# yanzq95/DHD

Hardware: AMD Instinct MI355X
Metric: samples/sec (6-cam fwd+bwd) DHD-S view-transform hot path (higher is better)
Workload: dtype f32

## Files before the change

dhd_amd/csrc/sfa_stage.hip:

```cpp
#include <stdlib.h>

#include <type_traits>

#include "sfa_gemm_cu.h"
#include "sfa_half.h"
#include "sfa_mfma.h"

using namespace dhd_sfa;

namespace {

constexpr int kEwBlock = 256;
constexpr int kPlaneChunks = 4;
constexpr int kPwBlock = 256;
constexpr int kPwStep = 16;
constexpr int kWgBlock = 512;
constexpr int kWgStride = 33;
constexpr int kWgWorkers = 256;
__host__ __device__ inline long long wg_first_step(long long n, long long w, long long W) { return n * w / W; }
__host__ __device__ inline int wg_owner(long long n, long long s, long long W) { return (int)(((s + 1) * W + n - 1) / n) - 1; }
inline int wgrad_blocks(int c) { const int ot = c == 128 ? 128 : 256; return (c / ot) * (c / ot); }
inline int wgrad_workers(int c) { const int nob = wgrad_blocks(c); return kWgWorkers / nob > 0 ? kWgWorkers / nob : 1; }
constexpr int kBwdFoldDefault = 3;

__device__ __forceinline__ float block_sum(float v, float* sm) {
  v = group_sum(v, DHD_WAVE);
  const int lane = threadIdx.x & 63, wv = threadIdx.x >> 6;
  __syncthreads();
  if (lane == 0) sm[wv] = v;
  __syncthreads();
  float t = 0.f;
  for (int k = 0; k < (int)(blockDim.x / DHD_WAVE); ++k) t += sm[k];
  return t;
}

template <class TS> constexpr bool kHalfStorage = !std::is_same_v<TS, float>;
template <class TS> constexpr bool kStreamAll = kHalfStorage<TS>;
template <class TS> constexpr int kWideInFlight = kHalfStorage<TS> ? 2 : 1;
template <class TS> constexpr bool kFoldPairwise = !kHalfStorage<TS>;

template <int N> __device__ __forceinline__ void chunk_range(int hw, int* lo, int* hi) {
  static_assert(N == 4 || N == 8, "16 bytes of float32 or of a half type");
  const int n = hw >> (N == 8 ? 3 : 2), per = (n + kPlaneChunks - 1) / kPlaneChunks;
  *lo = blockIdx.x * per;
  *hi = min(n, *lo + per);
}

template <class TO, int N> struct IoVec {
  static constexpr bool k16 = N == kVec16<TO>;
  static_assert(k16 || (N == 4 && sizeof(TO) == 2), "16 bytes, or four elements of a half type");
  using raw = std::conditional_t<k16, raw16<TO>, u32x2>;
  static __device__ __forceinline__ raw ld(const TO* base, size_t i) { return __builtin_nontemporal_load(reinterpret_cast<const raw*>(base) + i); }
  static __device__ __forceinline__ void widen(raw w, float* v) {
    if constexpr (k16) {
      widen16<TO>(w, v);
    } else {
      const f32x2 a = Pair<TO>::widen(w.x), b = Pair<TO>::widen(w.y);
      v[0] = a.x; v[1] = a.y; v[2] = b.x; v[3] = b.y;
    }
  }
  static __device__ __forceinline__ void store(TO* base, size_t i, const float* v) {
    if constexpr (k16) {
      Vec16<TO, true>::store(base, i, v);
    } else {
      typedef TO t4 __attribute__((ext_vector_type(4)));
      const t4 h = {(TO)v[0], (TO)v[1], (TO)v[2], (TO)v[3]};
      __builtin_nontemporal_store(h, reinterpret_cast<t4*>(base) + i);
    }
  }
};

template <int N> __device__ __forceinline__ float tree_sum(const float* v) {
  if constexpr (N == 4) return (v[0] + v[1]) + (v[2] + v[3]);
  else return tree_sum<N / 2>(v) + tree_sum<N / 2>(v + N / 2);
}

template <class TS> __device__ __forceinline__ float fold_sum(float acc, const float* a) {
  if constexpr (kFoldPairwise<TS>) return acc + tree_sum<kVec16<TS>>(a);
#pragma unroll
  for (int j = 0; j < kVec16<TS>; ++j) acc += a[j];
  return acc;
}
template <class TS, class D> __device__ __forceinline__ float fold_dot(float acc, const float* a, D d) {
  if constexpr (kFoldPairwise<TS>) {
    static_assert(kVec16<TS> == 4, "the pairwise fold is written for four elements");
    return acc + ((a[0] * d(0) + a[1] * d(1)) + (a[2] * d(2) + a[3] * d(3)));
  }
#pragma unroll
  for (int j = 0; j < kVec16<TS>; ++j) acc = fmaf(a[j], d(j), acc);
  return acc;
}

template <int K, class Load, class Body> __device__ __forceinline__ void for_each_vector(int lo, int hi, Load load, Body body) {
  int i = lo + threadIdx.x;
  if constexpr (K == 2) {
    for (; i + kEwBlock < hi; i += 2 * kEwBlock) {
      const auto u = load(i), w = load(i + kEwBlock);
      body(u, i);
      body(w, i + kEwBlock);
    }
    if (i < hi) body(load(i), i);
  } else {
    for (; i < hi; i += kEwBlock) body(load(i), i);
  }
}


template <class TS>
__device__ __forceinline__ void plane_mean_block(const TS* __restrict__ x, float* __restrict__ part, int hw, float* sm) {
  constexpr int N = kVec16<TS>;
  using X = Vec16<TS, true>;
  const size_t plane = blockIdx.y;
  const TS* p = x + plane * hw;
  int lo, hi;
  chunk_range<N>(hw, &lo, &hi);
  float a0 = 0.f, a1 = 0.f;
  int i = lo + threadIdx.x;
  for (; i + kEwBlock < hi; i += 2 * kEwBlock) {
    float v[N], w[N];
    X::load(p, i, v);
    X::load(p, (size_t)i + kEwBlock, w);
    a0 += tree_sum<N>(v);
    a1 += tree_sum<N>(w);
  }
  if (i < hi) {
    float v[N];
    X::load(p, i, v);
    a0 += tree_sum<N>(v);
  }
  const float tot = block_sum(a0 + a1, sm);
  if (threadIdx.x == 0) part[plane * kPlaneChunks + blockIdx.x] = tot;
}

__global__ __launch_bounds__(kEwBlock) void plane_mean_kernel(const float* __restrict__ x, float* __restrict__ part, int hw) {
  __shared__ float sm[kEwBlock / DHD_WAVE];
  plane_mean_block(x, part, hw, sm);
}

constexpr int kFcBlock = 1024;
__global__ __launch_bounds__(kFcBlock) void fc_forward_kernel(const float* __restrict__ part, const float* __restrict__ w1,
                                                              const float* __restrict__ b1, const float* __restrict__ w2,
                                                              const float* __restrict__ b2, float* __restrict__ s,
                                                              float* __restrict__ hbuf, float* __restrict__ a,
                                                              float* __restrict__ tab, int c, int r, int hw,
                                                              int* __restrict__ ticks, int n_ticks) {
  extern __shared__ float sh[];
  if (blockIdx.x == 0)
    for (int i = threadIdx.x; i < n_ticks; i += kFcBlock) ticks[i] = 0;
  float* ss = sh;
  float* hh = sh + 2 * c;
  const int b = blockIdx.x, c2 = 2 * c;
  for (int i = threadIdx.x; i < c2; i += kFcBlock) {
    const float* q = part + ((size_t)b * c2 + i) * kPlaneChunks;
    float v = ((q[0] + q[1]) + (q[2] + q[3])) / (float)hw;
    ss[i] = v;
    s[(size_t)b * c2 + i] = v;
  }
  __syncthreads();
  const int lane = threadIdx.x & 63, wv = threadIdx.x >> 6;
  for (int j0 = wv * 4; j0 < r; j0 += 4 * (kFcBlock / DHD_WAVE)) {
    float acc[4] = {0.f, 0.f, 0.f, 0.f};
    for (int i = lane; i < c2; i += DHD_WAVE) {
      const float sv = ss[i];
#pragma unroll
      for (int q = 0; q < 4; ++q)
        if (j0 + q < r) acc[q] = fmaf(w1[(size_t)(j0 + q) * c2 + i], sv, acc[q]);
    }
#pragma unroll
    for (int q = 0; q < 4; ++q) {
      const float t = group_sum(acc[q], DHD_WAVE);
      if (lane == 0 && j0 + q < r) {
        const float v = fmaxf(t + b1[j0 + q], 0.f);
        hh[j0 + q] = v;
        hbuf[(size_t)b * r + j0 + q] = v;
      }
    }
// ... 1337 lines not shown
      constexpr int OT = decltype(ot_c)::value;
      if constexpr (!std::is_same<TS, float>::value) {
        const size_t shmem = (size_t)2 * 4 * 2 * (OT / 32) * 64 * 16;
        return launch_lds<pw_wgrad_h_kernel<TS, OT, V::two, V::relu>>(grid, block, shmem, shmem, st, a0, a1, acoef, a_bs, b0, b1, bcoef,
                                                                     b_bs, partial, c, hw, b, workers);
      } else if (p.wgrad == Wgrad::w3) {
        const size_t shmem = (size_t)2 * 2 * 2 * (OT / 32) * 2 * 64 * 16;
        if (fold.mode != 0) {
          if (nob != 1 || fold.mode != (V::two ? 2 : 1)) return (int)DHD_EUNSUPPORTED;
          return launch_lds<pw_wgrad3_kernel<OT, false, V::two, V::relu, V::two ? 2 : 1>>(grid, block, shmem, shmem, st, a0, a1, acoef, a_bs, b0, b1,
                                                                                         bcoef, b_bs, partial, c, hw, b, workers, fold.aux,
                                                                                         fold.mean, fold.rows);
        }
        return launch_lds<pw_wgrad3_kernel<OT, true, V::two, V::relu>>(grid, block, shmem, shmem, st, a0, a1, acoef, a_bs, b0, b1, bcoef,
                                                                      b_bs, partial, c, hw, b, workers, static_cast<const float*>(nullptr),
                                                                      static_cast<const float*>(nullptr), static_cast<float*>(nullptr));
      } else if (p.wgrad == Wgrad::w6) {
        const size_t shmem = (size_t)2 * 2 * (OT / 32) * 3 * 64 * 16;
        return launch_lds<pw_wgrad6_kernel<OT, true, V::two, V::relu>>(grid, block, shmem, shmem, st, a0, a1, acoef, a_bs, b0, b1, bcoef,
                                                                      b_bs, partial, c, hw, b, workers);
      } else {
        const size_t shmem = (size_t)4 * OT * kWgStride * sizeof(float);
        return launch_lds<pw_wgrad_kernel<OT, true, V::two, V::relu>>(grid, block, shmem, shmem, st, a0, a1, acoef, a_bs, b0, b1, bcoef,
                                                                     b_bs, partial, c, hw, b, workers);
      }
    };
    return ot == 128 ? run(IntC<128>{}) : run(IntC<256>{});
  });
  if (rc != DHD_OK) return rc;
  const int n = c * c;
  hipLaunchKernelGGL(wgrad_reduce_kernel, dim3(dhd_cdiv(n, DHD_WAVE)), dim3(kEwBlock), 0, st, partial, gw, n, workers);
  DHD_LAUNCH_CHECK();
  return DHD_OK;
}

template <class TS>
int launch_mean_pack(const Plan& p, const TS* x, const float* w1, const float* w2, void* const dst[4], float* mean_part, int b,
                     int c, int hw, hipStream_t st) {
  const int blocks_each = dhd_cdiv((c / 32) * (c / 16) * 64, kEwBlock);
  if (p.pack == Pack::cu || p.pack == Pack::res || p.pack == Pack::cuh) {
    PackJob job;
    job.w[0] = w1; job.w[1] = w2;
    for (int i = 0; i < 4; ++i) job.dst[i] = static_cast<u32x4*>(dst[i]);
    job.c = c; job.nt = p.nt; job.cob = p.cob; job.cu = p.pack == Pack::cu ? 1 : 0;
    job.blocks_each = blocks_each;
    const dim3 grid(kPlaneChunks, b * 2 * c + dhd_cdiv(4 * blocks_each, kPlaneChunks));
    hipLaunchKernelGGL(plane_mean_pack_kernel<TS>, grid, dim3(kEwBlock), 0, st, x, mean_part, hw, b * 2 * c, job);
    DHD_LAUNCH_CHECK();
    return DHD_OK;
  }
  if constexpr (std::is_same_v<TS, float>) {
    hipLaunchKernelGGL(plane_mean_kernel, dim3(kPlaneChunks, b * 2 * c), dim3(kEwBlock), 0, st, x, mean_part, hw);
    DHD_LAUNCH_CHECK();
    for (int i = 0; i < 4; ++i) {
      const float* wi = i & 1 ? w2 : w1;
      if (p.pack == Pack::six)
        hipLaunchKernelGGL(pack_weight6_kernel, dim3(blocks_each), dim3(kEwBlock), 0, st, wi, i >> 1, static_cast<u32x4*>(dst[i]), c, p.cot);
      else
        hipLaunchKernelGGL(pack_weight_kernel, dim3(dhd_cdiv(c * c, kEwBlock)), dim3(kEwBlock), 0, st, wi, i >> 1, static_cast<float*>(dst[i]),
                           c, p.cot);
      DHD_LAUNCH_CHECK();
    }
    return DHD_OK;
  }
  return DHD_EINVAL;
}

template <class TS, class TO>
int stage_forward(const Plan& p, const TS* x, const dhd_sfa_weights* w, TO* out, void* saved, void* scratch, int b, int c, int hw,
                  int lo, int hi, double* sync, hipStream_t st) {
  const int r = w->hidden;
  const SavedLayout S = saved_layout(b, c, hw, r, p.storage);
  const ScratchLayout T = scratch_layout(b, c, hw, r, p.storage);
  char* sv = static_cast<char*>(saved);
  char* sc = static_cast<char*>(scratch);
  auto SF = [&](size_t off) { return reinterpret_cast<float*>(sv + off); };
  auto TF = [&](size_t off) { return reinterpret_cast<float*>(sc + off); };
  TS* y1 = reinterpret_cast<TS*>(sv + S.y1);
  TS* y2 = reinterpret_cast<TS*>(sv + S.y2);
  float* stat_part = p.fused_stats ? TF(T.stat_part) : nullptr;
  const dim3 planes(kPlaneChunks, b * c), per_ch(dhd_cdiv(c, kEwBlock));
  const size_t cs = (size_t)c * hw;
  int stat_rows = 0, rc;
  struct Bn {
    const float *shift, *gamma, *beta;
    float *run_mean, *run_var;
    float momentum, eps;
    long long* batches;
    float *mean, *rstd, *scsh;
    double* loc;
  };
  const Bn bn1 = {w->conv1_b, w->bn1_w, w->bn1_b, w->bn1_mean, w->bn1_var, w->momentum1, w->eps1,
                  reinterpret_cast<long long*>(w->bn1_batches), SF(S.mean1), SF(S.rstd1), SF(S.scsh1), reinterpret_cast<double*>(sv + S.loc1)};
  const Bn bn2 = {w->conv2_b, w->bn2_w, w->bn2_b, w->bn2_mean, w->bn2_var, w->momentum2, w->eps2,
                  reinterpret_cast<long long*>(w->bn2_batches), SF(S.mean2), SF(S.rstd2), SF(S.scsh2), reinterpret_cast<double*>(sv + S.loc2)};
  auto publish = [&](const Bn& n, float* tab) {
    hipLaunchKernelGGL(bn_stats_finalize_kernel, dim3(c / 4), dim3(kEwBlock), 0, st, TF(T.stat_part), stat_rows, n.shift, n.gamma, n.beta,
                       n.run_mean, n.run_var, n.momentum, n.eps, n.mean, n.rstd, n.scsh, tab, b, c, hw, sync, n.loc, nullptr, nullptr);
  };
  auto coef = [&](const Bn& n, const TS* y, float* tab) {
    if (!w->training) {
      hipLaunchKernelGGL(bn_eval_coef_kernel, per_ch, dim3(kEwBlock), 0, st, n.gamma, n.beta, n.run_mean, n.run_var, n.eps, n.mean, n.rstd,
                         n.scsh, tab, b, c);
    } else if (p.fused_stats) {
      hipLaunchKernelGGL(bn_stats_finalize_kernel, dim3(c / 4), dim3(kEwBlock), 0, st, TF(T.stat_part), stat_rows, n.shift, n.gamma, n.beta,
                         n.run_mean, n.run_var, n.momentum, n.eps, n.mean, n.rstd, n.scsh, tab, b, c, hw, nullptr, nullptr, sync, n.batches);
    } else if constexpr (std::is_same<TS, float>::value) {
      hipLaunchKernelGGL(moments_kernel, planes, dim3(kEwBlock), 0, st, y, TF(T.part), c, hw);
      hipLaunchKernelGGL(bn_train_finalize_kernel, per_ch, dim3(kEwBlock), 0, st, TF(T.part), b * kPlaneChunks, y, hw, n.gamma, n.beta,
                         n.run_mean, n.run_var, n.momentum, n.eps, n.mean, n.rstd, n.scsh, tab, b, c, hw, n.batches);
    }
  };
  if (sync && !p.fused_stats) return DHD_EUNSUPPORTED;

  if (lo <= 0) {
    void* const dst[4] = {sc + T.wp1, sc + T.wp2, sv + S.wp1t, sv + S.wp2t};
    rc = launch_mean_pack(p, x, w->conv1_w, w->conv2_w, dst, TF(T.mean_part), b, c, hw, st);
    if (rc != DHD_OK) return rc;
    hipLaunchKernelGGL(fc_forward_kernel, dim3(b), dim3(kFcBlock), (size_t)(2 * c + r) * sizeof(float), st, TF(T.mean_part), w->fc1_w,
                       w->fc1_b, w->fc2_w, w->fc2_b, SF(S.s), SF(S.h), SF(S.a1), SF(S.tab_a), c, r, hw, reinterpret_cast<int*>(sv + S.tick),
                       2 * c + kTickWords);
    DHD_LAUNCH_CHECK();
    rc = launch_gemm(p, GemmCall<TS>{kConv1, x, x + cs, 2 * cs, c, SF(S.tab_a), sc + T.wp1, w->conv1_b, nullptr, stat_part, y1},
                     b, c, hw, st, &stat_rows);
    if (rc != DHD_OK) return rc;
    if (sync) {
      publish(bn1, SF(S.tab1));
      DHD_LAUNCH_CHECK();
    }
  }
  if (hi <= 0) return DHD_OK;
  if (lo <= 1) {
    coef(bn1, y1, SF(S.tab1));
    DHD_LAUNCH_CHECK();
    rc = launch_gemm(p, GemmCall<TS>{kConv2, y1, nullptr, cs, c, SF(S.tab1), sc + T.wp2, w->conv2_b,
                                     reinterpret_cast<unsigned*>(sv + S.mask), stat_part, y2},
                     b, c, hw, st, &stat_rows);
    if (rc != DHD_OK) return rc;
    if (sync) {
      publish(bn2, TF(T.tab_g2));
      DHD_LAUNCH_CHECK();
    }
  }
  if (hi <= 1) return DHD_OK;
  coef(bn2, y2, TF(T.tab_g2));
  hipLaunchKernelGGL((blend2_bn_kernel<TS, TO>), planes, dim3(kEwBlock), 0, st, x, SF(S.a1), y2, SF(S.scsh2), out, c, hw);
  DHD_LAUNCH_CHECK();
  return DHD_OK;
}

int bwd_fold_mode() {
  static const int mode = [] {
    const char* e = getenv("DHD_SFA_BWD_FOLD");
    return e != nullptr && e[0] >= '0' && e[0] <= '3' && e[1] == 0 ? e[0] - '0' : kBwdFoldDefault;
  }();
  return mode;
}

template <class TS, class TO>
int stage_backward(const Plan& p, const TS* x, const dhd_sfa_weights* w, const void* saved, const TO* gout, TO* gx,
                   const dhd_sfa_grads* grads, void* scratch, int b, int c, int hw, int lo, int hi, double* sync, hipStream_t st) {
  const int r = w->hidden;
  const SavedLayout S = saved_layout(b, c, hw, r, p.storage);
  const ScratchLayout T = scratch_layout(b, c, hw, r, p.storage);
  char* sv = const_cast<char*>(static_cast<const char*>(saved));
  char* sc = static_cast<char*>(scratch);
  auto SF = [&](size_t off) { return reinterpret_cast<float*>(sv + off); };
  auto TF = [&](size_t off) { return reinterpret_cast<float*>(sc + off); };
  const TS* y1 = reinterpret_cast<const TS*>(sv + S.y1);
  const TS* y2 = reinterpret_cast<const TS*>(sv + S.y2);
  TS* g2 = reinterpret_cast<TS*>(sc + T.g2);
  TS* g1 = reinterpret_cast<TS*>(sc + T.g1);
  TS* du = reinterpret_cast<TS*>(sc + T.du);
  unsigned* mask = reinterpret_cast<unsigned*>(sv + S.mask);
  int* tick = reinterpret_cast<int*>(sv + S.tick);
  const dim3 planes(kPlaneChunks, b * c), per_ch(dhd_cdiv(c, kEwBlock));
  const size_t cs = (size_t)c * hw;
  int rc;
  const BnTail tail2 = {sync ? nullptr : tick, w->bn2_w, SF(S.mean2), SF(S.rstd2), TF(T.tab_g2), grads->bn2_w, grads->bn2_b,
                        grads->conv2_b, w->training, b, hw};
  const BnTail tail1 = {sync ? nullptr : tick + c, w->bn1_w, SF(S.mean1), SF(S.rstd1), TF(T.tab_g1), grads->bn1_w, grads->bn1_b,
                        grads->conv1_b, w->training, b, hw};
  auto coef_out = [&](const BnTail& t) {
    hipLaunchKernelGGL(bn_backward_coef_kernel, per_ch, dim3(kEwBlock), 0, st, TF(T.part), t.gamma, t.mean, t.rstd, w->training, t.tab,
                       t.dgamma, t.dbeta, t.dbias, b, c, hw, sync, nullptr, nullptr, nullptr);
  };
  auto coef_in = [&](const BnTail& t, size_t loc, const float* bias) {
    hipLaunchKernelGGL(bn_backward_coef_kernel, per_ch, dim3(kEwBlock), 0, st, TF(T.part), t.gamma, t.mean, t.rstd, w->training, t.tab,
                       t.dgamma, t.dbeta, t.dbias, b, c, hw, nullptr, sync, reinterpret_cast<const double*>(sv + loc), bias);
  };
  if (sync && !p.fused_stats) return DHD_EUNSUPPORTED;
  int fold = 0;
  const int fold_workers = wgrad_workers(c);
  if constexpr (std::is_same_v<TS, float>) {
    const size_t plane = (size_t)b * cs * sizeof(float);
    if (p.gemm == Gemm::cu && p.wgrad == Wgrad::w3 && sync == nullptr && wgrad_blocks(c) == 1 && (size_t)fold_workers * 2 * c * sizeof(float) <= plane &&
        (size_t)(fold_workers + b) * c * sizeof(float) <= plane)
      fold = bwd_fold_mode();
  }
  float* rows1 = reinterpret_cast<float*>(du);
  float* rows2 = reinterpret_cast<float*>(g2);

  if (lo <= 0) {
    hipLaunchKernelGGL((blend2_bn_bwd_kernel<TS, TO>), planes, dim3(kEwBlock), 0, st, x, SF(S.a1), y2, SF(S.scsh2), SF(S.mean2), gout, g2, TF(T.part),
                       TF(T.da1), c, hw, tail2);
    if (sync) coef_out(tail2);
    DHD_LAUNCH_CHECK();
  }
  if (hi <= 0) return DHD_OK;
  if (lo <= 1) {
    if (sync) coef_in(tail2, S.loc2, w->conv2_b);
    DHD_LAUNCH_CHECK();
  }
  if (lo <= 1 && (fold & 1)) {
    if constexpr (std::is_same_v<TS, float>) {
      rc = launch_gemm(p, GemmCall<TS>{kDgrad2, g2, y2, cs, c, TF(T.tab_g2), sv + S.wp2t, nullptr, mask, nullptr, g1, y1, SF(S.scsh1), CuBlend{}, 0, g2},
                       b, c, hw, st);
      if (rc != DHD_OK) return rc;
      rc = launch_wgrad<TS>(p, kConv2, g2, nullptr, nullptr, cs, y1, nullptr, SF(S.tab1), cs, TF(T.wpart), grads->conv2_w, b, c, hw, st,
                            WgradFold{1, g1, SF(S.mean1), rows1});
      if (rc != DHD_OK) return rc;
      const BnRowsJob j1 = {tail1.gamma, tail1.mean, tail1.rstd, tail1.tab, tail1.dgamma, tail1.dbeta, tail1.dbias, w->training, b, hw};
      hipLaunchKernelGGL(bn_backward_rows_kernel, dim3(c / 4), dim3(kEwBlock), 0, st, rows1, fold_workers, j1, c);
      DHD_LAUNCH_CHECK();
    }
  } else if (lo <= 1) {
    rc = launch_wgrad<TS>(p, kConv2, g2, y2, TF(T.tab_g2), cs, y1, nullptr, SF(S.tab1), cs, TF(T.wpart), grads->conv2_w, b, c, hw, st);
    if (rc != DHD_OK) return rc;
    rc = launch_gemm(p, GemmCall<TS>{kDgrad2, g2, y2, cs, c, TF(T.tab_g2), sv + S.wp2t, nullptr, mask, nullptr, g1, y1, SF(S.scsh1)},
                     b, c, hw, st);
    if (rc != DHD_OK) return rc;
    hipLaunchKernelGGL(pair_sums_kernel<TS>, planes, dim3(kEwBlock), 0, st, g1, y1, SF(S.mean1), TF(T.part), c, hw, tail1);
    if (sync) coef_out(tail1);
    DHD_LAUNCH_CHECK();
  }
  if (hi <= 1) return DHD_OK;
  if (sync) coef_in(tail1, S.loc1, w->conv1_b);
  DHD_LAUNCH_CHECK();
  if (fold & 2) {
    if constexpr (std::is_same_v<TS, float>) {
      rc = launch_gemm(p, GemmCall<TS>{kDgrad1, g1, y1, cs, c, TF(T.tab_g1), sv + S.wp1t, nullptr, nullptr, nullptr, du, nullptr, nullptr, CuBlend{}, 0, g1},
                       b, c, hw, st);
      if (rc != DHD_OK) return rc;
      rc = launch_wgrad<TS>(p, kConv1, g1, nullptr, nullptr, cs, x, x + cs, SF(S.tab_a), 2 * cs, TF(T.wpart), grads->conv1_w, b, c, hw, st,
                            WgradFold{2, du, nullptr, rows2});
      if (rc != DHD_OK) return rc;
      hipLaunchKernelGGL(fc_backward_kernel, dim3(b), dim3(kEwBlock), (size_t)(c + r + kEwBlock) * sizeof(float), st, TF(T.da1), rows2,
                         SF(S.a1), SF(S.h), w->fc1_w, w->fc2_w, TF(T.dpre2), TF(T.dh), TF(T.ds), c, r, fold_workers, (hw + 31) / 32);
    }
  } else {
    rc = launch_wgrad<TS>(p, kConv1, g1, y1, TF(T.tab_g1), cs, x, x + cs, SF(S.tab_a), 2 * cs, TF(T.wpart), grads->conv1_w, b, c, hw, st);
    if (rc != DHD_OK) return rc;
    rc = launch_gemm(p, GemmCall<TS>{kDgrad1, g1, y1, cs, c, TF(T.tab_g1), sv + S.wp1t, nullptr, nullptr, nullptr, du}, b, c, hw, st);
    if (rc != DHD_OK) return rc;
    hipLaunchKernelGGL(blend1_da_kernel<TS>, planes, dim3(kEwBlock), 0, st, x, du, TF(T.da2), c, hw);
    hipLaunchKernelGGL(fc_backward_kernel, dim3(b), dim3(kEwBlock), (size_t)(c + r + kEwBlock) * sizeof(float), st, TF(T.da1), TF(T.da2),
                       SF(S.a1), SF(S.h), w->fc1_w, w->fc2_w, TF(T.dpre2), TF(T.dh), TF(T.ds), c, r, 0, 0);
  }
  const int n_fc = r * 2 * c + c * r + r + c;
  const FcGradJob fcj = {TF(T.dpre2), TF(T.dh), SF(S.h), SF(S.s), grads->fc1_w, grads->fc1_b, grads->fc2_w, grads->fc2_b, b, r};
  const int fc_rows = dhd_cdiv(dhd_cdiv(n_fc, kEwBlock), kPlaneChunks);
  const dim3 planes_fc(kPlaneChunks, b * c + fc_rows);
  hipLaunchKernelGGL((stage_gx_kernel<TS, TO>), planes_fc, dim3(kEwBlock), 0, st, SF(S.a1), y2, SF(S.scsh2), gout, du, TF(T.ds), gx, c, hw, fc_rows, fcj);
  DHD_LAUNCH_CHECK();
  return DHD_OK;
}

inline bool infer_form_exists(const Plan& p, int form) {
  switch (form) {
    case DHD_SFA_INFER_AUTO: case DHD_SFA_INFER_UNFUSED: return true;
    case DHD_SFA_INFER_TWO_PASS: return p.gemm == Gemm::cu || p.gemm == Gemm::cuh;
    case DHD_SFA_INFER_ONE_PASS: return p.gemm == Gemm::cuh;
    default: return false;
  }
}
inline int infer_resolve(const Plan& p, int form) {
  if (form != DHD_SFA_INFER_AUTO) return form;
  if (infer_form_exists(p, DHD_SFA_INFER_ONE_PASS)) return DHD_SFA_INFER_ONE_PASS;
  return infer_form_exists(p, DHD_SFA_INFER_TWO_PASS) ? DHD_SFA_INFER_TWO_PASS : DHD_SFA_INFER_UNFUSED;
}

struct InferLayout {
  size_t wp1, wp2, mean_part, s, h, a1, tab_a, mean1, rstd1, scsh1, tab1, mean2, rstd2, scsh2, tab2, y1, total;
};
inline InferLayout infer_layout(int b, int c, int hw, int r, int storage, bool with_y1) {
  const bool half = storage != DHD_F32;
  const size_t cc = (size_t)c * c;
  InferLayout L;
  size_t o = 0;
  auto take = [&](size_t bytes) { size_t at = o; o += (bytes + 255) & ~(size_t)255; return at; };
  auto f = [&](size_t n) { return take(n * sizeof(float)); };
  L.wp1 = take(half ? 2 * cc : 8 * cc); L.wp2 = take(half ? 2 * cc : 8 * cc);
  L.mean_part = f((size_t)b * 2 * c * kPlaneChunks);
  L.s = f((size_t)b * 2 * c); L.h = f((size_t)b * r); L.a1 = f((size_t)b * c); L.tab_a = f((size_t)b * 3 * c);
  L.mean1 = f(c); L.rstd1 = f(c); L.scsh1 = f(2 * c); L.tab1 = f((size_t)b * 3 * c);
  L.mean2 = f(c); L.rstd2 = f(c); L.scsh2 = f(2 * c); L.tab2 = f((size_t)b * 3 * c);
  L.y1 = take(with_y1 ? (size_t)b * c * hw * (half ? 2 : 4) : 0);
  L.total = o;
  return L;
}

inline size_t infer_scratch_total(const Plan& p, int form, int b, int c, int hw, int r) {
  const int f = infer_resolve(p, form);
  if (f != DHD_SFA_INFER_UNFUSED) return infer_layout(b, c, hw, r, p.storage, f == DHD_SFA_INFER_TWO_PASS).total;
  return saved_layout(b, c, hw, r, p.storage).total + scratch_layout(b, c, hw, r, p.storage).total;
}

template <class TS>
int launch_onepass(const TS* x, const OnePassArgs& A, TS* out, int b, int c, int hw, hipStream_t st) {
  const int max_b = onepass_max_batch(c);
  if (max_b < 1) return DHD_EUNSUPPORTED;
  const int nwt = (hw + kCuhTile - 1) / kCuhTile;
  int cus = cu_count();
  if (cus <= 0) cus = 256;
  for (int b0 = 0; b0 < b; b0 += max_b) {
    const int nb = b - b0 < max_b ? b - b0 : max_b;
    const long total = (long)nb * nwt;
    const int grid = (int)(total < cus ? total : cus);
    OnePassArgs a = A;
    a.tab_a += (size_t)b0 * 3 * c;
    a.a1 += (size_t)b0 * c;
    const TS* xi = x + (size_t)b0 * 2 * c * hw;
    TS* oi = out + (size_t)b0 * c * hw;
    const size_t shmem = onepass_lds_bytes(c, nb);
    const int rc = c == 256 ? launch_lds<sfa_onepass_h_kernel<TS, 16>>(dim3(grid), dim3(kOnePassWaves * 64), shmem, kLdsBytes, st, xi, a, oi, hw, nb)
                            : launch_lds<sfa_onepass_h_kernel<TS, 8>>(dim3(grid), dim3(kOnePassWaves * 64), shmem, kLdsBytes, st, xi, a, oi, hw, nb);
    if (rc != DHD_OK) return rc;
  }
  return DHD_OK;
}

template <class TS, class TO>
int stage_infer(const Plan& p, const TS* x, const dhd_sfa_weights* w, TO* out, void* scratch, int b, int c, int hw, int form,
                hipStream_t st) {
  const int r = w->hidden;
  char* sc = static_cast<char*>(scratch);
  form = infer_resolve(p, form);
  if (form == DHD_SFA_INFER_UNFUSED)
    return stage_forward<TS, TO>(p, x, w, out, sc, sc + saved_layout(b, c, hw, r, p.storage).total, b, c, hw, 0, 2, nullptr, st);
  const InferLayout L = infer_layout(b, c, hw, r, p.storage, form == DHD_SFA_INFER_TWO_PASS);
  auto F = [&](size_t off) { return reinterpret_cast<float*>(sc + off); };
  TS* y1 = reinterpret_cast<TS*>(sc + L.y1);
  const size_t cs = (size_t)c * hw;
  void* const dst[4] = {sc + L.wp1, sc + L.wp2, nullptr, nullptr};
  int rc = launch_mean_pack(p, x, w->conv1_w, w->conv2_w, dst, F(L.mean_part), b, c, hw, st);
  if (rc != DHD_OK) return rc;
  hipLaunchKernelGGL(fc_forward_kernel, dim3(b), dim3(kFcBlock), (size_t)(2 * c + r) * sizeof(float), st, F(L.mean_part), w->fc1_w, w->fc1_b,
                     w->fc2_w, w->fc2_b, F(L.s), F(L.h), F(L.a1), F(L.tab_a), c, r, hw, static_cast<int*>(nullptr), 0);
  DHD_LAUNCH_CHECK();
  const BnEvalJob j1 = {w->bn1_w, w->bn1_b, w->bn1_mean, w->bn1_var, w->eps1, F(L.mean1), F(L.rstd1), F(L.scsh1), F(L.tab1)};
  const BnEvalJob j2 = {w->bn2_w, w->bn2_b, w->bn2_mean, w->bn2_var, w->eps2, F(L.mean2), F(L.rstd2), F(L.scsh2), F(L.tab2)};
  hipLaunchKernelGGL(bn_eval_coef2_kernel, dim3(dhd_cdiv(c, kEwBlock), 2), dim3(kEwBlock), 0, st, j1, j2, b, c);
  DHD_LAUNCH_CHECK();
  if (form == DHD_SFA_INFER_ONE_PASS) {
    if constexpr (std::is_same<TS, float>::value) {
      return DHD_EUNSUPPORTED;
    } else {
      const OnePassArgs A = {F(L.tab_a), F(L.tab1), w->conv1_b, w->conv2_b, F(L.a1), F(L.scsh2), reinterpret_cast<const u32x4*>(sc + L.wp1),
                             reinterpret_cast<const u32x4*>(sc + L.wp2)};
      return launch_onepass<TS>(x, A, reinterpret_cast<TS*>(out), b, c, hw, st);
    }
  }
  rc = launch_gemm(p, GemmCall<TS>{kConv1, x, x + cs, 2 * cs, c, F(L.tab_a), sc + L.wp1, w->conv1_b, nullptr, nullptr, y1}, b, c, hw, st);
  if (rc != DHD_OK) return rc;
  return launch_gemm(p, GemmCall<TS>{kConv2Blend, y1, nullptr, cs, c, F(L.tab1), sc + L.wp2, w->conv2_b, nullptr, nullptr, nullptr, nullptr,
                                     nullptr, CuBlend{x, F(L.a1), F(L.scsh2), out}, w->io_dtype},
                     b, c, hw, st);
// ... 153 lines not shown
```

Measured before the change: 2709.

## Fuse conv2 dgrad and weight-gradient into single paired MFMA kernel in backward

Adds a pw_pair_kernel that, per 32-pixel step, computes the blended conv2 output gradient, performs the data-gradient GEMM with split-bf16 MFMA, applies the BN1 ReLU mask and accumulates row statistics, and simultaneously accumulates the conv2 weight-gradient partials from the same LDS-staged tiles. This replaces the separate dgrad GEMM and wgrad launches in the fold path, so g2 and y1 are read once instead of twice. Fold mode default becomes 7 to enable it. The kernel splits input channels across two blocks per worker and needs a follow-up partial reduction, so it adds large LDS use and a one-block-per-CU occupancy limit.

```diff
diff --git a/dhd_amd/csrc/sfa_gemm_pair.h b/dhd_amd/csrc/sfa_gemm_pair.h
--- /dev/null
+++ b/dhd_amd/csrc/sfa_gemm_pair.h
@@ -0,0 +1,307 @@
+#pragma once
+#include "sfa_gemm_cu.h"
+
+namespace dhd_sfa {
+
+constexpr int kPairWorkers = 128;
+constexpr int kPairGrid = 2 * kPairWorkers;
+constexpr int kPairPatchPitch = 36;
+
+struct PairSlot { int worker, half; };
+__host__ __device__ inline PairSlot pair_slot(int block) {
+  PairSlot s;
+  s.worker = (block >> 4) * 8 + (block & 7);
+  s.half = (block >> 3) & 1;
+  return s;
+}
+
+__host__ __device__ inline int pair_d_write(int co, int p, int part) {
+  const int q = p >> 2, e = p & 3;
+  return (((((co >> 5) * 2 + part) * 2 + (e >> 1)) * 64 + 16 * ((co >> 3) & 3) + q + 8 * (e & 1)) << 4) + 8 * ((co >> 2) & 1);
+}
+__host__ __device__ inline int pair_d_read(int ks, int part, int nt, int lane) { return ((((ks * 2 + part) * 2 + nt) * 64) + lane) << 4; }
+__host__ __device__ inline int pair_a_write(int c, int co, int q, int part) {
+  const int kk = q >> 2, h = (q >> 1) & 1;
+  return ((((kk * (c / 32) + (co >> 5)) * 2 + part) * 64 + ((co & 31) ^ (2 * kk + h)) + 32 * h) << 4) + 8 * (q & 1);
+}
+__host__ __device__ inline int pair_a_read(int c, int kk, int tile, int part, int lane) {
+  return (((kk * (c / 32) + tile) * 2 + part) * 64 + (lane ^ (2 * kk + (lane >> 5)))) << 4;
+}
+__host__ __device__ inline int pair_b_write(int c, int ci, int q, int part) {
+  const int kk = q >> 2, h = (q >> 1) & 1;
+  return ((((kk * (c / 64) + (ci >> 5)) * 2 + part) * 64 + ((ci & 31) ^ ((2 * kk + h) << 1)) + 32 * h) << 4) + 8 * (q & 1);
+}
+__host__ __device__ inline int pair_b_read(int c, int kk, int tile, int part, int lane) {
+  return (((kk * (c / 64) + tile) * 2 + part) * 64 + (lane ^ ((2 * kk + (lane >> 5)) << 1))) << 4;
+}
+
+inline size_t pair_lds_bytes(int c) {
+  return (size_t)128 * c + 128 * c + 64 * c + (size_t)(c / 32) * 16 * kPairPatchPitch * sizeof(float) + (size_t)3 * c * sizeof(float);
+}
+
+struct PairArgs {
+  const float* g;
+  const float* y;
+  const float* coef;
+  const u32x4* wp;
+  const float* b;
+  const float* b_scsh;
+  const float* b_mean;
+  float* out;
+  float* partial;
+  float* rows;
+  int hw, nb;
+};
+
+__device__ __forceinline__ f32x4 mfma16_bf16(u32x4 a, u32x4 b, f32x4 c) {
+  return __builtin_amdgcn_mfma_f32_16x16x32_bf16(__builtin_bit_cast(bf16x8, a), __builtin_bit_cast(bf16x8, b), c, 0, 0, 0);
+}
+
+template <int C, int AUX, class FirstStep>
+__global__ __launch_bounds__(2 * C, 1) void pw_pair_kernel(PairArgs a) {
+  static_assert(C == 128 || C == 256, "C/32 waves, C/64 weight-gradient tiles per wave");
+  constexpr int KS = C / 32, KCN = C / 16, HALF = C / 2;
+  constexpr int TCO = C / 32, TCI = C / 64;
+  constexpr int TA = C / 128, TB = 2, WCI = TCI / TB;
+  constexpr int DIMG = 128 * C, AIMG = 128 * C, BIMG = 64 * C;
+  extern __shared__ __attribute__((aligned(16))) unsigned char pair_lds[];
+  unsigned char* const dimg = pair_lds;
+  unsigned char* const aimg = pair_lds + DIMG;
+  unsigned char* const bimg = pair_lds + DIMG + AIMG;
+  const int tid = threadIdx.x, lane = tid & 63;
+  const int wv = __builtin_amdgcn_readfirstlane(tid >> 6);
+  const int g = lane >> 3, q = lane & 7;
+  float* const patch = reinterpret_cast<float*>(pair_lds + DIMG + AIMG + BIMG) + wv * (16 * kPairPatchPitch);
+  const PairSlot slot = pair_slot((int)blockIdx.x);
+  const int cib = slot.half * HALF;
+  const int hw = a.hw, sps = (hw + 31) >> 5;
+  const long long n_steps = (long long)a.nb * sps;
+  const int first = (int)FirstStep{}(n_steps, slot.worker, kPairWorkers);
+  const int count = (int)FirstStep{}(n_steps, slot.worker + 1, kPairWorkers) - first;
+  const int row_bytes = hw * 4;
+  const unsigned in_bytes = (unsigned)((size_t)C * hw * sizeof(float));
+
+  u32x4 wh[KS], wm[KS];
+  {
+    const int row = cib + 16 * wv + (lane & 15), kq = lane >> 4;
+#pragma unroll
+    for (int ks = 0; ks < KS; ++ks) {
+      const u32x4* src = a.wp + ((size_t)((row >> 5) * KCN + 2 * ks + (kq >> 1)) * 2) * 64 + (row & 31) + 32 * (kq & 1);
+      wh[ks] = src[0];
+      wm[ks] = src[64];
+    }
+  }
+  const int co0 = 32 * wv + 4 * g;
+  float* const cf_lds = reinterpret_cast<float*>(pair_lds + DIMG + AIMG + BIMG) + (C / 32) * (16 * kPairPatchPitch);
+  for (int i = tid; i < 3 * C; i += 2 * C) cf_lds[i] = a.coef[i];
+  float bsc[2], bsh[2], bmu[2];
+#pragma unroll
+  for (int k = 0; k < 2; ++k) {
+    const int ch = cib + 16 * wv + g + 8 * k;
+    bsc[k] = a.b_scsh[ch];
+    bsh[k] = a.b_scsh[C + ch];
+    bmu[k] = a.b_mean[ch];
+  }
+  const int lda_voff = (co0 * hw + 4 * q) * 4;
+  const int ldb_voff = ((cib + 16 * wv + g) * hw + 4 * q) * 4;
+  int aw[4], bw[2];
+#pragma unroll
+  for (int j = 0; j < 4; ++j) aw[j] = pair_a_write(C, co0 + j, q, 0);
+#pragma unroll
+  for (int k = 0; k < 2; ++k) bw[k] = pair_b_write(C, 16 * wv + g + 8 * k, q, 0);
+  const int dw = pair_d_write(co0, 4 * q, 0);
+  const int a_rd = (lane ^ (lane >> 5)) << 4, b_rd = (lane ^ ((lane >> 5) << 1)) << 4;
+
+  f32x16 acc[TA][TB];
+#pragma unroll
+  for (int i = 0; i < TA; ++i)
+#pragma unroll
+    for (int j = 0; j < TB; ++j)
+#pragma unroll
+      for (int e = 0; e < 16; ++e) acc[i][j][e] = 0.f;
+  float s1[2] = {0.f, 0.f}, s2[2] = {0.f, 0.f};
+
+  f32x4 rg[4], ry[4], rb[2];
+  auto issue = [&](int s) {
+    const int b = s / sps, p0 = (s - b * sps) * 32;
+    const __amdgpu_buffer_rsrc_t sg = __builtin_amdgcn_make_buffer_rsrc(const_cast<float*>(a.g + (size_t)b * C * hw), 0, in_bytes, 0x00020000);
+    const __amdgpu_buffer_rsrc_t sy = __builtin_amdgcn_make_buffer_rsrc(const_cast<float*>(a.y + (size_t)b * C * hw), 0, in_bytes, 0x00020000);
+    const __amdgpu_buffer_rsrc_t sb = __builtin_amdgcn_make_buffer_rsrc(const_cast<float*>(a.b + (size_t)b * C * hw), 0, in_bytes, 0x00020000);
+    const bool okq = p0 + 4 * q < hw;
+    const int va = okq ? lda_voff : lda_voff - 16 * q, vb = okq ? ldb_voff : ldb_voff - 16 * q;
+#pragma unroll
+    for (int j = 0; j < 4; ++j) {
+      rg[j] = __builtin_bit_cast(f32x4, __builtin_amdgcn_raw_buffer_load_b128(sg, va, j * row_bytes + p0 * 4, AUX));
+      ry[j] = __builtin_bit_cast(f32x4, __builtin_amdgcn_raw_buffer_load_b128(sy, va, j * row_bytes + p0 * 4, AUX));
+    }
+#pragma unroll
+    for (int k = 0; k < 2; ++k) rb[k] = __builtin_bit_cast(f32x4, __builtin_amdgcn_raw_buffer_load_b128(sb, vb, 8 * k * row_bytes + p0 * 4, AUX));
+  };
+
+  __builtin_amdgcn_s_waitcnt(0x0F70);
+  cu_lds_barrier();
+  if (count > 0) {
+    issue(first);
+    {
+      const __amdgpu_buffer_rsrc_t ro = __builtin_amdgcn_make_buffer_rsrc(a.out, 0, 16, 0x00020000);
+      store_b128_guarded<0>(u32x4{0u, 0u, 0u, 0u}, ro, 0x7ffffff0, 0);
+      store_b128_guarded<0>(u32x4{0u, 0u, 0u, 0u}, ro, 0x7ffffff0, 0);
+    }
+  }
+  for (int it = 0; it < count; ++it) {
+    const int s = first + it;
+    const int b = s / sps, p0 = (s - b * sps) * 32;
+    const bool okq = p0 + 4 * q < hw;
+    float v[4][4];
+    {
+      const f32x4 c0 = *reinterpret_cast<const f32x4*>(cf_lds + co0);
+      const f32x4 c1 = *reinterpret_cast<const f32x4*>(cf_lds + C + co0);
+      const f32x4 c2 = *reinterpret_cast<const f32x4*>(cf_lds + 2 * C + co0);
+#pragma unroll
+      for (int e = 0; e < 4; ++e)
+#pragma unroll
+        for (int j = 0; j < 4; ++j) {
+          float tv = fmaf(c0[j], rg[j][e], c2[j]);
+          tv = fmaf(c1[j], ry[j][e], tv);
+          v[e][j] = okq ? tv : 0.f;
+        }
+    }
+    f32x4 yk[2];
+    unsigned pass[2];
+    float z[2][4];
+#pragma unroll
+    for (int k = 0; k < 2; ++k) {
+      yk[k] = rb[k];
+      pass[k] = 0;
+#pragma unroll
+      for (int e = 0; e < 4; ++e) {
+        const float zr = fmaxf(fmaf(bsc[k], rb[k][e], bsh[k]), 0.f);
+        pass[k] |= min(__float_as_uint(zr), 1u) << e;
+        z[k][e] = okq ? zr : 0.f;
+      }
+    }
+    __builtin_amdgcn_sched_barrier(0);
+    issue(first + min(it + 1, count - 1));
+    __builtin_amdgcn_sched_barrier(0);
+    unsigned h01[4], m01[4], h23[4], m23[4];
+#pragma unroll
+    for (int e = 0; e < 4; ++e) {
+      split2_hm(v[e][0], v[e][1], h01[e], m01[e]);
+      split2_hm(v[e][2], v[e][3], h23[e], m23[e]);
+      const int off = dw + (((e >> 1) * 64 + 8 * (e & 1)) << 4);
+      *reinterpret_cast<u32x2*>(dimg + off) = u32x2{h01[e], h23[e]};
+      *reinterpret_cast<u32x2*>(dimg + off + 2048) = u32x2{m01[e], m23[e]};
+    }
+    {
+      constexpr unsigned LO = 0x05040100u, HI = 0x07060302u;
+#pragma unroll
+      for (int j = 0; j < 4; ++j) {
+        const unsigned* hs = j < 2 ? h01 : h23;
+        const unsigned* ms = j < 2 ? m01 : m23;
+        const unsigned sel = (j & 1) ? HI : LO;
+        const u32x2 hq = {__builtin_amdgcn_perm(hs[1], hs[0], sel), __builtin_amdgcn_perm(hs[3], hs[2], sel)};
+        const u32x2 mq = {__builtin_amdgcn_perm(ms[1], ms[0], sel), __builtin_amdgcn_perm(ms[3], ms[2], sel)};
+        *reinterpret_cast<u32x2*>(aimg + aw[j]) = hq;
+        *reinterpret_cast<u32x2*>(aimg + aw[j] + 1024) = mq;
+      }
+    }
+#pragma unroll
+    for (int k = 0; k < 2; ++k) {
+      unsigned zh01, zm01, zh23, zm23;
+      split2_hm(z[k][0], z[k][1], zh01, zm01);
+      split2_hm(z[k][2], z[k][3], zh23, zm23);
+      *reinterpret_cast<u32x2*>(bimg + bw[k]) = u32x2{zh01, zh23};
+      *reinterpret_cast<u32x2*>(bimg + bw[k] + 1024) = u32x2{zm01, zm23};
+    }
+    cu_lds_barrier();
+
+    f32x4 dacc[2] = {{0.f, 0.f, 0.f, 0.f}, {0.f, 0.f, 0.f, 0.f}};
+#pragma unroll
+    for (int ks = 0; ks < KS; ++ks)
+#pragma unroll
+      for (int nt = 0; nt < 2; ++nt) {
+        const u32x4 bh = *reinterpret_cast<const u32x4*>(dimg + pair_d_read(ks, 0, nt, lane));
+        const u32x4 bm = *reinterpret_cast<const u32x4*>(dimg + pair_d_read(ks, 1, nt, lane));
+        dacc[nt] = mfma16_bf16(wm[ks], bh, dacc[nt]);
+        dacc[nt] = mfma16_bf16(wh[ks], bm, dacc[nt]);
+        dacc[nt] = mfma16_bf16(wh[ks], bh, dacc[nt]);
+      }
+    {
+      const int wco = wv / WCI, wci = wv % WCI;
+#pragma unroll
+      for (int k2 = 0; k2 < 2; ++k2) {
+        u32x4 fb[TB][2];
+#pragma unroll
+        for (int j = 0; j < TB; ++j)
+#pragma unroll
+          for (int t = 0; t < 2; ++t) fb[j][t] = *reinterpret_cast<const u32x4*>(bimg + ((((k2 * TCI + TB * wci + j) * 2 + t) * 64) << 4) + (b_rd ^ (k2 << 6)));
+#pragma unroll
+        for (int i = 0; i < TA; ++i) {
+          u32x4 fa[2];
+#pragma unroll
+          for (int t = 0; t < 2; ++t) fa[t] = *reinterpret_cast<const u32x4*>(aimg + ((((k2 * TCO + TA * wco + i) * 2 + t) * 64) << 4) + (a_rd ^ (k2 << 5)));
+#pragma unroll
+          for (int j = 0; j < TB; ++j) acc[i][j] = mfma_bf16(fa[1], fb[j][0], acc[i][j]);
+#pragma unroll
+          for (int j = 0; j < TB; ++j) acc[i][j] = mfma_bf16(fa[0], fb[j][1], acc[i][j]);
+#pragma unroll
+          for (int j = 0; j < TB; ++j) acc[i][j] = mfma_bf16(fa[0], fb[j][0], acc[i][j]);
+        }
+      }
+    }
+    {
+      const int col = lane & 15, prow = 4 * (lane >> 4);
+#pragma unroll
+      for (int nt = 0; nt < 2; ++nt)
+#pragma unroll
+        for (int i = 0; i < 4; ++i) patch[(prow + i) * kPairPatchPitch + 4 * (col & 7) + 2 * nt + (col >> 3)] = dacc[nt][i];
+      const __amdgpu_buffer_rsrc_t ro = __builtin_amdgcn_make_buffer_rsrc(a.out + (size_t)b * C * hw, 0, in_bytes, 0x00020000);
+      const int voff = okq ? ldb_voff : 0x7ffffff0;
+#pragma unroll
+      for (int k = 0; k < 2; ++k) {
+        f32x4 o = *reinterpret_cast<const f32x4*>(patch + (g + 8 * k) * kPairPatchPitch + 4 * q);
+#pragma unroll
+        for (int e = 0; e < 4; ++e) o[e] = __int_as_float(__float_as_int(o[e]) & __builtin_amdgcn_sbfe((int)pass[k], e, 1));
+        const f32x4 y1 = yk[k];
+        const float mu = bmu[k];
+        const float t1 = (o.x + o.y) + (o.z + o.w);
+        const float t2 = (o.x * (y1.x - mu) + o.y * (y1.y - mu)) + (o.z * (y1.z - mu) + o.w * (y1.w - mu));
+        s1[k] += okq ? t1 : 0.f;
+        s2[k] += okq ? t2 : 0.f;
+        store_b128_guarded<0>(__builtin_bit_cast(u32x4, o), ro, voff, 8 * k * row_bytes + p0 * 4);
+      }
+    }
+    cu_lds_barrier();
+  }
+
+  {
+    const int wco = wv / WCI, wci = wv % WCI;
+    float* po = a.partial + (size_t)slot.worker * C * C;
+#pragma unroll
+    for (int i = 0; i < TA; ++i)
+#pragma unroll
+      for (int j = 0; j < TB; ++j)
+#pragma unroll
+        for (int e = 0; e < 16; ++e) {
+          const int co = 32 * (TA * wco + i) + (e & 3) + 8 * (e >> 2) + 4 * (lane >> 5);
+          const int ci = cib + 32 * (TB * wci + j) + (lane & 31);
+          po[(size_t)co * C + ci] = acc[i][j][e];
+        }
+  }
+#pragma unroll
+  for (int k = 0; k < 2; ++k) {
+    float v1 = s1[k], v2 = s2[k];
+#pragma unroll
+    for (int m = 1; m < 8; m <<= 1) {
+      v1 += __shfl_xor(v1, m, DHD_WAVE);
+      v2 += __shfl_xor(v2, m, DHD_WAVE);
+    }
+    if (q == 0) {
+      float* row = a.rows + (size_t)slot.worker * 2 * C + cib + 16 * wv + g + 8 * k;
+      row[0] = v1;
+      row[C] = v2;
+    }
+  }
+}
+
+}
diff --git a/dhd_amd/csrc/sfa_stage.hip b/dhd_amd/csrc/sfa_stage.hip
--- a/dhd_amd/csrc/sfa_stage.hip
+++ b/dhd_amd/csrc/sfa_stage.hip
@@ -3,6 +3,7 @@
 #include <type_traits>
 
 #include "sfa_gemm_cu.h"
+#include "sfa_gemm_pair.h"
 #include "sfa_half.h"
 #include "sfa_mfma.h"
 
@@ -19,9 +20,12 @@
 constexpr int kWgWorkers = 256;
 __host__ __device__ inline long long wg_first_step(long long n, long long w, long long W) { return n * w / W; }
 __host__ __device__ inline int wg_owner(long long n, long long s, long long W) { return (int)(((s + 1) * W + n - 1) / n) - 1; }
+struct WgFirstStep {
+  __host__ __device__ long long operator()(long long n, long long w, long long W) const { return wg_first_step(n, w, W); }
+};
 inline int wgrad_blocks(int c) { const int ot = c == 128 ? 128 : 256; return (c / ot) * (c / ot); }
 inline int wgrad_workers(int c) { const int nob = wgrad_blocks(c); return kWgWorkers / nob > 0 ? kWgWorkers / nob : 1; }
-constexpr int kBwdFoldDefault = 3;
+constexpr int kBwdFoldDefault = 7;
 
 __device__ __forceinline__ float block_sum(float v, float* sm) {
   v = group_sum(v, DHD_WAVE);
@@ -1665,9 +1669,22 @@
 int bwd_fold_mode() {
   static const int mode = [] {
     const char* e = getenv("DHD_SFA_BWD_FOLD");
-    return e != nullptr && e[0] >= '0' && e[0] <= '3' && e[1] == 0 ? e[0] - '0' : kBwdFoldDefault;
+    return e != nullptr && e[0] >= '0' && e[0] <= '7' && e[1] == 0 ? e[0] - '0' : kBwdFoldDefault;
   }();
   return mode;
+}
+
+int launch_pair(const PairArgs& a, float* gw, int c, hipStream_t st) {
+  const size_t shmem = pair_lds_bytes(c);
+  int rc;
+  if (c == 256) rc = launch_lds<pw_pair_kernel<256, 2, WgFirstStep>>(dim3(kPairGrid), dim3(512), shmem, shmem, st, a);
+  else if (c == 128) rc = launch_lds<pw_pair_kernel<128, 2, WgFirstStep>>(dim3(kPairGrid), dim3(256), shmem, shmem, st, a);
+  else return DHD_EUNSUPPORTED;
+  if (rc != DHD_OK) return rc;
+  const int n = c * c;
+  hipLaunchKernelGGL(wgrad_reduce_kernel, dim3(dhd_cdiv(n, DHD_WAVE)), dim3(kEwBlock), 0, st, a.partial, gw, n, kPairWorkers);
+  DHD_LAUNCH_CHECK();
+  return DHD_OK;
 }
 
 template <class TS, class TO>
@@ -1725,7 +1742,17 @@
     if (sync) coef_in(tail2, S.loc2, w->conv2_b);
     DHD_LAUNCH_CHECK();
   }
-  if (lo <= 1 && (fold & 1)) {
+  if (lo <= 1 && (fold & 4)) {
+    if constexpr (std::is_same_v<TS, float>) {
+      rc = launch_pair(PairArgs{g2, y2, TF(T.tab_g2), reinterpret_cast<const u32x4*>(sv + S.wp2t), y1, SF(S.scsh1), SF(S.mean1), g1, TF(T.wpart),
+                                rows1, hw, b},
+                       grads->conv2_w, c, st);
+      if (rc != DHD_OK) return rc;
+      const BnRowsJob j1 = {tail1.gamma, tail1.mean, tail1.rstd, tail1.tab, tail1.dgamma, tail1.dbeta, tail1.dbias, w->training, b, hw};
+      hipLaunchKernelGGL(bn_backward_rows_kernel, dim3(c / 4), dim3(kEwBlock), 0, st, rows1, kPairWorkers, j1, c);
+      DHD_LAUNCH_CHECK();
+    }
+  } else if (lo <= 1 && (fold & 1)) {
     if constexpr (std::is_same_v<TS, float>) {
       rc = launch_gemm(p, GemmCall<TS>{kDgrad2, g2, y2, cs, c, TF(T.tab_g2), sv + S.wp2t, nullptr, mask, nullptr, g1, y1, SF(S.scsh1), CuBlend{}, 0, g2},
                        b, c, hw, st);
```

After: 2830, median of 6. 4.5% higher.
